# will-rowe/groot

Hardware: AMD Instinct MI355X
Metric: Mreads/s aligned (higher is better)
Workload: dtype u64

## Files before the change

### groot_amd/csrc/hip/ctx.hpp

```cpp
#pragma once

#include <hip/hip_runtime.h>

#include <algorithm>
#include <array>
#include <atomic>
#include <cstdlib>
#include <deque>
#include <map>
#include <memory>
#include <string>
#include <thread>
#include <vector>

#include "device_types.hpp"

using namespace groot;


template <class T> struct DevBuf {
    T *p = nullptr;
    size_t n = 0;
    hipError_t alloc(size_t count)
    {
// ... 245 lines not shown
    DevBuf<uint64_t> d_mask;
    DevBuf<DeviceCounters> d_ctr;
    PinBuf<DeviceCounters> h_ctr;
    PinBuf<groot_trav> h_trav;
    DevBuf<groot_ctrav> d_ctrav;
    PinBuf<groot_ctrav> h_ctrav;
    PinBuf<uint8_t> h_mask;
    PinBuf<uint32_t> h_ckpt;
    DevBuf<uint8_t> d_cmask;
    DevBuf<uint32_t> d_mwords, d_moff, d_ckpt;
    uint32_t n_trav = 0, copied = 0;
    uint64_t n_mask_bytes = 0, copied_bytes = 0;
    bool host_results = false;
    hipEvent_t ev_seed = nullptr;
    hipEvent_t ev_walk = nullptr;
    hipEvent_t ev_h2d0 = nullptr, ev_h2d = nullptr, ev_compute = nullptr, ev_ctr = nullptr, ev_d2h0 = nullptr, ev_d2h = nullptr;
    hipEvent_t ev[14]{};
    groot_counts counts{};
    int status = GROOT_OK;
    std::string status_msg;
    groot_stage_ms ms{};
    SlotCounters ct;
    const uint8_t *seq() const { return input == IN_DEVICE ? ext_seq : d_seq.p; }
    const uint64_t *off() const { return input == IN_DEVICE ? ext_off : d_off.p; }
};

struct WorkSet {
    DevBuf<uint32_t> seed_count, seed_win, perm, perm_count, trav_cnt, tab_idx;
    DevBuf<uint32_t> perm2;
    DevBuf<uint4> packed;
    DevBuf<ReadRec> read_rec;
    DevBuf<uint4> vitem, split_list;
    DevBuf<uint32_t> vcount;
    DevBuf<groot_trav> trav_first;
    DevBuf<uint64_t> mask_first, sketches;
    DevBuf<groot_trav> ovf_trav;
    DevBuf<uint64_t> ovf_mask;
    DevBuf<uint32_t> ovf_cnt;
    hipEvent_t ev_free = nullptr;
    bool used = false;
    Slot *owner = nullptr;
    uint64_t ticket = 0;
};

struct groot_ctx {
    int device = 0;
    std::string err;
    groot_params prm{};
    Knobs kn;
    uint32_t s = 0, k = 0, max_k = 0, l_max = 0, pw_view = 0, pw = 0, n_windows = 0, max_q = 0, band_hash_bits = 0;
    hipEvent_t h2d_last = nullptr;
    Slot *newest = nullptr;
    hipEvent_t last_compute = nullptr;
    hipStream_t own_stream = nullptr, stream = nullptr, astream = nullptr, tstream = nullptr, own_tstream = nullptr, h2d_stream = nullptr, d2h_stream = nullptr;
    bool profiling = false;

    DevBuf<uint32_t> graph_win_end;
    DevBuf<uint4> cn_pre;
    DevBuf<uint64_t> node_l2b;
    DevBuf<uint32_t> win_prefix, edges, win_graph, cn_node,
        band_keys, band_ids;
    DevBuf<ExactEntry> band_hash;
    DevBuf<uint8_t> band_sig;
    DevBuf<uint32_t> band_run;
    DevBuf<uint8_t> bases, q_k, q_l;
    DevBuf<uint16_t> q_min_eq;
    DevBuf<uint64_t> win_sketch;
    DevBuf<unsigned char> node_rec;
// ... 111 lines not shown
```

### groot_amd/csrc/hip/device_types.hpp

```cpp
#pragma once

#include <cstdint>

#include <hip/hip_runtime.h>

#include "groot_hip.h"

namespace groot {

constexpr int kBlock = 256;
constexpr uint32_t kEmpty = 0xFFFFFFFFu;

enum : uint32_t {
    kFlagShortRead = 1u,
    kFlagLongRead = 2u,
    kFlagSeedOverflow = 4u,
    kFlagTravOverflow = 8u,
    kFlagOrdOverflow = 16u,
    kFlagOvfOverflow = 32u,
    kFlagQOverflow = 64u,
};

constexpr uint32_t kIncrCap = 8;
constexpr uint32_t kIncrCapBig = 2048;
// ... 137 lines not shown

struct SeedArgs {
    DeviceIndex ix;
    const uint8_t *seq;
    const uint64_t *seq_off;
    uint32_t n_reads, max_read_len;
    uint32_t lds_read_bytes;
    uint32_t seed_slots;
    uint32_t *seed_count;
    uint32_t *seed_win;
    uint64_t *sketch_out;
    uint32_t *sort_key;
    uint32_t sort_span_bits;
    uint32_t sort_span_shift;
    ReadRec *read_rec;
    uint32_t *q_seen;
    uint32_t *trav_cnt;
    unsigned long long *shards;
    uint32_t *tab_idx;
    uint32_t *tab_hist;
    uint32_t *lsh_list, *lsh_count;
    uint64_t *lsh_sketch;
    uint32_t *dfs_list, *dfs_count;
    uint32_t *long_list, *long_count;
    uint4 *packed;
    uint32_t packed_q;
    uint32_t *todo_list;
    uint32_t *todo_count;
    uint32_t lsh_defer_rows, lsh_cap;
    uint32_t list_stride_dw;
    DeviceCounters *ctr;
};

struct AlignArgs {
    DeviceIndex ix;
    const uint8_t *seq;
    const uint64_t *seq_off;
    uint32_t n_reads, first_read_id;
    uint32_t seed_slots;
    const uint32_t *seed_count;
    const uint32_t *seed_win;
    const uint32_t *perm;
    const ReadRec *read_rec;
    uint32_t no_align, update_weights;
    const void *node_rec;
    uint32_t *attempts;
    groot_trav *trav_first;
    uint64_t *mask_first;
    uint32_t *trav_cnt;
    groot_trav *ovf_trav;
    uint64_t *ovf_mask;
    uint32_t *ovf_cnt;
    uint32_t ovf_cap;
    uint64_t *stk_hdr;
    uint64_t *stk_mask;
    uint32_t n_threads, stk_depth;
    uint32_t lds_stride_dw;
    uint32_t *incr_cnt, *incr_win;
    uint32_t incr_cap;
    uint32_t head_lanes;
    uint32_t round_lanes;
    const uint4 *vitem;
    const uint32_t *vcount;
    uint32_t vcap;
    const uint32_t *n_perm;
    const uint32_t *rest;
    uint32_t rest_lo;
    uint32_t refill;
    DeviceCounters *ctr;
};

struct alignas(16) LeanNode {
    uint32_t seq_off;
    uint32_t seq_len;
    uint32_t deg_kids;
    uint32_t pad;
    uint32_t edges[4];
    uint64_t first32;
    uint64_t mask[3];
};
static_assert(sizeof(LeanNode) == 64, "lean node record is one 64-byte line");
constexpr uint32_t kLeanNo = 0x80000000u;
struct alignas(16) LeanExt {
    uint64_t b[7];
    uint64_t pad;
};
static_assert(sizeof(LeanExt) == 64, "lean node extension is one 64-byte line");
constexpr uint32_t kLeanMaxLen = 256;

struct LeanArgs {
    const LeanNode *nodes;
    const LeanExt *ext;
    const uint32_t *bases2;
    const uint4 *cn_pre2;
    const uint64_t *node_l2b;
    const uint8_t *win_ok;
    const WinRec *win_rec;
    const uint32_t *q_row;
    const uint8_t *seq;
    const uint4 *packed;
    uint32_t packed_q;
    const uint32_t *perm;
    const ReadRec *read_rec;
    uint32_t n_reads, first_read_id, n_windows, k;
    uint32_t update_weights;
    uint32_t lds_stride_dw;
    uint32_t max_len;
    uint32_t *attempts;
    groot_trav *trav_first;
    uint64_t *mask_first;
    uint32_t *trav_cnt;
    uint32_t *left;
    uint32_t *left_cnt;
    uint4 *stk;
    groot_trav *ovf_trav;
    uint64_t *ovf_mask;
    uint32_t *ovf_cnt;
    uint32_t ovf_cap;
    DeviceCounters *ctr;
    const uint4 *path_node;
    const uint32_t *path_text;
    const uint32_t *path_tag;
    const uint32_t *path_nodes;
    const uint64_t *path_tab;
    uint4 *hold;
};

__host__ __device__ inline uint32_t lean_stride_dw(uint32_t max_len) { return (((max_len + 15u) >> 4) + 15u) | 1u; }

#define GROOT_MULTI_SEED 0x90b45d39fb6da1faULL
__host__ __device__ __forceinline__ uint64_t sketch_hash_step(uint64_t h, uint64_t v)
{
    h = (h ^ v) * 0xff51afd7ed558ccdULL;
    return h ^ (h >> 29);
}
#define GROOT_SKETCH_HASH_INIT 0x9E3779B97F4A7C15ULL
__host__ __device__ __forceinline__ uint32_t sig5(uint64_t v) { return (uint32_t)((v * 0xD6E8FEB86659FD93ULL) >> 59); }
constexpr uint32_t kRowSlots = 24, kRowBytes = 16;
__host__ __device__ __forceinline__ uint64_t l2_bloom_bits(uint32_t code16)
{
    const uint32_t x = code16 * 0x9E3779B1u;
    return (1ull << (x >> 26)) | (1ull << ((x >> 20) & 63u));
}
// ... 43 lines not shown
```

### groot_amd/csrc/hip/groot_hip.hip

```cpp
#include <cstring>

#include <hip/hip_runtime.h>
#include <rocprim/rocprim.hpp>

#include <dlfcn.h>

#include <algorithm>
#include <cmath>
#include <cstdarg>
#include <cstdio>
#include <atomic>
#include <chrono>
#include <deque>
#include <iterator>
#include <array>
#include <map>
#include <tuple>
#include <memory>
#include <numeric>
#include <string>
#include <thread>
#include <vector>

#include "../common/cpus.hpp"
// ... 274 lines not shown
    auto sort = [&](void *tmp) {
        return small_blocks ? rocprim::radix_sort_pairs<OrderSortConfig>(tmp, tmp_bytes, c->sort_key.p, c->sort_key_out.p, c->perm_in.p, w->perm.p, s->n_reads,
                                                                         begin_bit, end_bit, c->stream)
                            : rocprim::radix_sort_pairs(tmp, tmp_bytes, c->sort_key.p, c->sort_key_out.p, c->perm_in.p, w->perm.p, s->n_reads, begin_bit, end_bit,
                                                        c->stream);
    };
    HIP_TRY(c, sort(nullptr));
    if (tmp_bytes > c->sort_tmp.n) {
        HIP_TRY(c, hipStreamSynchronize(c->stream));
        HIP_TRY(c, c->sort_tmp.alloc(tmp_bytes + tmp_bytes / 4));
    }
    HIP_TRY(c, sort(c->sort_tmp.p));
    return GROOT_OK;
}

static int launch_align_stage(groot_ctx *c, Slot *s, bool update_weights)
{
    WorkSet *w = &c->ws[s->set];
    AlignArgs a{};
    a.ix = c->dix;
    a.seq = s->seq();
    a.seq_off = s->off();
    a.n_reads = s->n_reads;
    a.first_read_id = s->first_read_id;
    a.seed_slots = c->seed_slots;
    a.seed_count = w->seed_count.p;
    a.seed_win = w->seed_win.p;
    a.perm = w->perm.p;
    a.read_rec = w->read_rec.p;
    a.no_align = c->prm.no_exact_align;
    a.update_weights = update_weights ? 1 : 0;
    a.attempts = c->attempts_ptr;
    a.node_rec = c->node_rec.p;
    a.trav_first = w->trav_first.p;
    a.mask_first = w->mask_first.p;
    a.trav_cnt = w->trav_cnt.p;
    a.ovf_trav = w->ovf_trav.p;
    a.ovf_mask = w->ovf_mask.p;
    a.ovf_cnt = w->ovf_cnt.p;
    a.ovf_cap = c->ovf_cap;
    if (c->vcap) { a.vitem = w->vitem.p; a.vcount = w->vcount.p; a.vcap = c->vcap; }
    a.stk_hdr = c->stk_hdr.p;
    a.stk_mask = c->stk_mask.p;
    uint32_t blocks = std::min<uint32_t>((s->n_reads + kBlock - 1) / kBlock, c->align_threads / kBlock);
    if (c->dfs_frac < kSparseBelow && c->dfs_frac * (double)s->n_reads < 16.0 * (double)(blocks * (kBlock / 64))) blocks = std::max(1u, blocks / 2);
    else if (error_batch(c, s) && blocks >= 4) blocks /= 2;
    if ((s->lean_used || s->path_used) && c->lean_left_frac < 0.25) {
        uint32_t want = (uint32_t)(c->lean_left_frac * 1.25 * (double)s->n_reads / 64.0 / (kBlock / 64)) + 1u;
        blocks = std::max(1u, std::min(blocks, std::max(want, c->n_cu)));
    }
    a.n_threads = blocks * kBlock;
    a.stk_depth = c->stk_depth;
    {
        const uint32_t stride = (2 + 4 * ((s->max_len + 27) / 16)) | 1u;
        a.lds_stride_dw = (size_t)kBlock * stride * 4 <= 64 * 1024 ? stride : 0;
    }
    if (c->tab_capture) {
        a.incr_cnt = c->incr_cnt.p; a.incr_win = c->incr_win.p; a.incr_cap = c->incr_cap;
        HIP_TRY(c, hipMemsetAsync(c->incr_cnt.p, 0, (size_t)s->n_reads * sizeof(uint32_t), c->tstream));
    }
    a.head_lanes = s->mixed_len ? 16u : 0u;
#ifndef GROOT_REFILL_ERR
#define GROOT_REFILL_ERR 48
#endif
#ifndef GROOT_REFILL_MIXED
#define GROOT_REFILL_MIXED 2
#endif
    a.refill = s->mixed_len ? (uint32_t)GROOT_REFILL_MIXED : (error_batch(c, s) ? (uint32_t)GROOT_REFILL_ERR : 64u);
#ifdef GROOT_WORK_COUNTERS
    if (const char *e = getenv("GROOT_DEV_ROUND")) a.round_lanes = (uint32_t)atoi(e);
#endif
    a.ctr = s->d_ctr.p;
    const bool first_pass = s->lean_used || s->path_used;
    const uint32_t lean_stride = lean_stride_dw(s->max_len);
    if (first_pass) {
        LeanArgs l{};
        l.nodes = c->lean_nodes.p; l.ext = c->lean_ext.p; l.bases2 = c->bases2.p; l.cn_pre2 = c->cn_pre2.p; l.win_ok = c->win_ok.p;
        l.win_rec = c->dix.win_rec; l.node_l2b = c->dix.node_l2b; l.q_row = c->q_row.p;
        l.seq = s->seq(); l.packed = s->packed_q ? w->packed.p : nullptr; l.packed_q = s->packed_q; l.perm = w->perm.p; l.read_rec = w->read_rec.p;
        l.n_reads = s->n_reads; l.first_read_id = s->first_read_id; l.n_windows = c->n_windows; l.k = c->k;
        l.update_weights = update_weights ? 1 : 0;
        l.lds_stride_dw = lean_stride; l.max_len = s->max_len;
        l.attempts = c->attempts_ptr;
        l.trav_first = w->trav_first.p; l.mask_first = w->mask_first.p; l.trav_cnt = w->trav_cnt.p;
        l.left = w->perm2.p; l.left_cnt = w->ovf_cnt.p + kOvfShards + 2; l.ctr = s->d_ctr.p;
        l.stk = c->lean_stk.p; l.ovf_trav = w->ovf_trav.p; l.ovf_mask = w->ovf_mask.p; l.ovf_cnt = w->ovf_cnt.p; l.ovf_cap = c->ovf_cap;
        const uint32_t lean_blocks = std::min<uint32_t>((s->n_reads + kBlock - 1) / kBlock, (uint32_t)(c->dfs_frac * 1.05 * (double)s->n_reads / kBlock) + 64u);
        if (s->path_used) {
            l.path_node = c->path_node.p; l.path_text = c->path_text.p; l.path_tag = c->path_tag.p; l.path_nodes = c->path_nodes.p; l.path_tab = c->path_tab.p;
            l.hold = c->path_hold.p;
            launch_align_path(c->pw, l, dim3(lean_blocks), c->astream);
        } else launch_align_lean(c->pw, l, dim3(lean_blocks), c->astream);
        HIP_TRY(c, hipGetLastError());
        a.perm = w->perm2.p;
        a.n_perm = l.left_cnt;
        a.rest = w->perm.p;
        a.rest_lo = lean_blocks * (uint32_t)kBlock;
        if (c->profiling) HIP_TRY(c, hipEventRecord(s->ev[13], c->astream));
        if (c->tstream != c->astream) {
            HIP_TRY(c, hipEventRecord(s->ev_walk, c->astream));
            HIP_TRY(c, hipStreamWaitEvent(c->tstream, s->ev_walk, 0));
        }
    }
    launch_align(c->pw, a, dim3(blocks), c->tstream);
    HIP_TRY(c, hipGetLastError());
    return GROOT_OK;
}

static int launch_order_stage(groot_ctx *c, Slot *s, bool update_weights)
{
    WorkSet *w = &c->ws[s->set];
    const uint32_t n = s->n_reads;
    size_t tmp_bytes = 0;
    if (c->vcap) hipLaunchKernelGGL(split_fix_kernel, dim3(256), dim3(kBlock), 0, c->tstream, w->split_list.p, w->vcount.p, w->vitem.p, w->trav_cnt.p, n, s->d_ctr.p,
                                    w->trav_first.p, w->mask_first.p, c->pw, s->first_read_id);
    HIP_TRY(c, rocprim::exclusive_scan(nullptr, tmp_bytes, w->trav_cnt.p, c->trav_off.p, 0u, n, rocprim::plus<uint32_t>(), c->tstream));
    if (tmp_bytes > c->scan_tmp.n) {
        HIP_TRY(c, hipStreamSynchronize(c->tstream));
        HIP_TRY(c, c->scan_tmp.alloc(tmp_bytes + tmp_bytes / 4));
    }
    HIP_TRY(c, rocprim::exclusive_scan(c->scan_tmp.p, tmp_bytes, w->trav_cnt.p, c->trav_off.p, 0u, n, rocprim::plus<uint32_t>(), c->tstream));
    OrderTabArgs ot{};
    if (c->dix.out_tab) {
        ot.tab_idx = w->tab_idx.p; ot.out_tab = c->dix.out_tab; ot.stride_q = c->dix.out_stride_q; ot.first_read_id = s->first_read_id;
        ot.update_weights = update_weights ? 1 : 0;
        ot.attempts = c->attempts_ptr; ot.q_row = c->q_row.p;
        ot.q_tab = c->dix.w - c->k + 1; ot.n_windows = c->n_windows;
    }
    if (c->profiling) HIP_TRY(c, hipEventRecord(s->ev[9], c->tstream));
    hipLaunchKernelGGL(order_first_kernel, dim3(std::min<uint32_t>((n + kBlock - 1) / kBlock, 2048u)), dim3(kBlock), 0, c->tstream, w->trav_first.p,
                       w->mask_first.p, c->trav_off.p, w->trav_cnt.p, n, s->d_trav.p, s->d_mask.p, s->trav_cap, c->pw,
                       c->pw_view, s->d_ctr.p, ot);
    if (c->profiling) HIP_TRY(c, hipEventRecord(s->ev[10], c->tstream));
    if (c->vcap) hipLaunchKernelGGL(order_split_kernel, dim3(std::min<uint32_t>((c->vcap + kBlock - 1) / kBlock, 256u)), dim3(kBlock), 0, c->tstream, w->vitem.p, w->vcount.p, c->vcap, w->trav_cnt.p,
                                    c->trav_off.p, w->trav_first.p, w->mask_first.p, n, s->first_read_id, s->d_trav.p, s->d_mask.p, s->trav_cap, c->pw, c->pw_view, s->d_ctr.p);
    hipLaunchKernelGGL(order_ovf_kernel, dim3((c->ovf_cap + kBlock - 1) / kBlock, kOvfShards), dim3(kBlock), 0, c->tstream,
                       w->ovf_trav.p, w->ovf_mask.p, w->ovf_cnt.p, c->ovf_cap, c->trav_off.p, s->first_read_id, s->d_trav.p,
                       s->d_mask.p, s->trav_cap, c->pw, c->pw_view, s->d_ctr.p, w->vitem.p, n, w->vcount.p);
    HIP_TRY(c, hipGetLastError());
    if (int rc = counters_assign(c, s)) return rc;
    if (!c->prm.results_on_device) {
        const dim3 g((s->trav_cap + kBlock - 1) / kBlock);
        hipLaunchKernelGGL(mask_words_kernel, g, dim3(kBlock), 0, c->tstream, s->d_trav.p, s->d_ctr.p, s->trav_cap, c->graph_words.p, (uint32_t)c->h_graph_words.size(),
                           s->d_mwords.p);
        size_t tb = 0;
        HIP_TRY(c, rocprim::exclusive_scan(nullptr, tb, s->d_mwords.p, s->d_moff.p, 0u, s->trav_cap, rocprim::plus<uint32_t>(), c->tstream));
        if (tb > c->scan_tmp.n) {
            HIP_TRY(c, hipStreamSynchronize(c->tstream));
            HIP_TRY(c, c->scan_tmp.alloc(tb + tb / 4));
        }
        HIP_TRY(c, rocprim::exclusive_scan(c->scan_tmp.p, tb, s->d_mwords.p, s->d_moff.p, 0u, s->trav_cap, rocprim::plus<uint32_t>(), c->tstream));
        hipLaunchKernelGGL(mask_compact_kernel, g, dim3(kBlock), 0, c->tstream, s->d_trav.p, s->d_mask.p, c->pw_view, s->d_ctr.p, s->trav_cap,
                           c->graph_words.p, (uint32_t)c->h_graph_words.size(), s->d_moff.p, s->d_cmask.p, s->d_ckpt.p);
        if (c->packed_travs) hipLaunchKernelGGL(trav_pack_kernel, g, dim3(kBlock), 0, c->tstream, s->d_trav.p, s->d_ctr.p, s->trav_cap, s->first_read_id, s->d_ctrav.p);
        HIP_TRY(c, hipGetLastError());
    }
    return GROOT_OK;
}


static int run_batch_async(groot_ctx *c, Slot *s, bool update_weights)
{
    WorkSet *w = &c->ws[s->set];
    if (w->used) HIP_TRY(c, hipStreamWaitEvent(c->stream, w->ev_free, 0));
    HIP_TRY(c, hipMemsetAsync(s->d_ctr.p, 0, sizeof(DeviceCounters), c->stream));
    if (c->kn.poison) {
        const size_t n = s->n_reads;
        HIP_TRY(c, hipMemsetAsync(w->seed_count.p, 0, n * sizeof(uint32_t), c->stream));
// ... 1255 lines not shown
```

### groot_amd/csrc/hip/kernels_align.hpp

```cpp
#pragma once

#include "kernels_common.hpp"

namespace groot {


enum : uint32_t { PH_FETCH, PH_SCAN, PH_DFS, PH_WAIT, PH_DONE, PH_FORK, PH_FORKWAIT, PH_JOIN };
#ifndef GROOT_FORK_MIN
#define GROOT_FORK_MIN 3
#endif
constexpr uint32_t kForkMin = GROOT_FORK_MIN;
constexpr uint32_t kClsHelper = 0x1000u;
constexpr uint32_t kCoopMin = 6;
constexpr uint32_t kCoopWant = 0xFFFFFFFEu;
#ifndef GROOT_COOP_MAX_ASK
#define GROOT_COOP_MAX_ASK 8
#endif
constexpr uint32_t kCoopMaxAsk = GROOT_COOP_MAX_ASK;
#ifndef GROOT_TL_LATE_US
#define GROOT_TL_LATE_US 3000
#endif
#ifndef GROOT_WAVE_CHUNK
#define GROOT_WAVE_CHUNK 128
#endif
// ... 670 lines not shown
            if (nb) {
                const uint8_t *gb = ix.bases + rec.seq_off() + coff;
                const uint64_t ga = coff == 0 ? rec.first8() : ld8(gb);
                ok = prefix_ok(ga, cur8, min(nb, 8u));
                for (uint32_t i = 8; ok && i < nb; i += 8)
                    ok = prefix_ok(ld8(gb + i), dfs_chunk(dist + i), nb - i);
            }
            bool backtrack = !ok;
            if (!ok) GROOT_EV(12);
            if (take > 8) GROOT_EV(11);
            if (take > 32) GROOT_EV(21);
            if (ok) {
                dist += nb; coff += nb;
                cur8 = dfs_chunk(dist);
                if (nb == take) {
                    GROOT_EV(13);
                    bool any = false;
#pragma unroll
                    for (int i = 0; i < PW; i++) { mask[i] &= rec.mask(i); any |= mask[i] != 0; }
                    const uint32_t rdeg = rec.deg();
                    if (dist == eff() || rdeg == 0) {
                        if (any && (cls & kClsHelper)) {
                            fk |= 1u << 12; sp = 0; emitted = 1;
                        } else if (any) {
                            GROOT_EV(14);
                            if (ord) GROOT_EV(19);
                            groot_trav t;
                            t.read_id = read_id; t.graph_id = g; t.node = node0; t.offset = noff0;
                            t.ord = (uint16_t)ord;
                            t.flags = (uint8_t)((rc ? GROOT_TRAV_RC : 0u) | (level == 3u ? GROOT_TRAV_START_CLIP : level == 4u ? GROOT_TRAV_END_CLIP : 0u) | (emitted == 0 ? GROOT_TRAV_FIRST : 0));
                            t.reserved = 0;
                            if (ord == 0) {
                                const uint32_t os = (cls & 0x400u) ? a.n_reads + slot : r;
                                a.trav_first[os] = t;
#pragma unroll
                                for (int i = 0; i < PW; i++) a.mask_first[(size_t)os * PW + i] = mask[i];
                            } else {
                                const uint32_t shard = blockIdx.x & (kOvfShards - 1);
                                const uint32_t slot = atomicAdd(&a.ovf_cnt[shard], 1u);
                                if (slot < a.ovf_cap) {
                                    const size_t o = (size_t)shard * a.ovf_cap + slot;
                                    a.ovf_trav[o] = t;
#pragma unroll
                                    for (int i = 0; i < PW; i++) a.ovf_mask[o * PW + i] = mask[i];
                                } else atomicOr(&a.ctr->flags, kFlagOvfOverflow);
                            }
                            if (ord >= 0xFFFFu) atomicOr(&a.ctr->flags, kFlagOrdOverflow);
                            ord++;
#pragma unroll
                            for (int i = 0; i < PW; i++) alns += __popcll(mask[i]);
                            emitted++;
                        }
                        backtrack = true;
                    } else if (!any) backtrack = true;
                    else {
                        const unsigned nextb = (unsigned)cur8 & 0xFF;
                        uint32_t first = kEmpty, more = kEmpty;
                        if (rdeg <= 4) {
#pragma unroll
                            for (int e = 3; e >= 0; e--) {
                                const unsigned cf1 = rec.child_first(e);
                                if ((uint32_t)e < rdeg && (cf1 == 'N' || cf1 == nextb)) { more = first; first = e; }
                            }
                        } else { first = 0; more = 1; }
                        if (first == kEmpty) backtrack = true;
                        else {
                            if (more != kEmpty) {
                                GROOT_EV(15);
                                const size_t si = (size_t)sp * a.n_threads + gtid;
// ... 120 lines not shown
```

### groot_amd/csrc/hip/kernels_lean.hpp

```cpp
#pragma once

#include "kernels_common.hpp"
#include "kernels_path.hpp"

namespace groot {


#ifndef GROOT_LEAN_WAVES
#define GROOT_LEAN_WAVES 5
#endif
constexpr int kLeanWaves = GROOT_LEAN_WAVES;
#ifndef GROOT_LEAN_MAX_ITER
#define GROOT_LEAN_MAX_ITER 96
#endif
constexpr uint32_t kLeanMaxIter = GROOT_LEAN_MAX_ITER;

__device__ __forceinline__ uint64_t lean_lowmask(int n) { return n <= 0 ? 0ull : (n >= 32 ? ~0ull : ((1ull << (2 * n)) - 1ull)); }
__device__ __forceinline__ uint32_t lean_revcomp16(uint32_t v)
{
    uint32_t r = __brev(v);
    r = ((r & 0xAAAAAAAAu) >> 1) | ((r & 0x55555555u) << 1);
    return r ^ 0xAAAAAAAAu;
}
__device__ __forceinline__ uint64_t lean_funnel(uint32_t x0, uint32_t x1, uint32_t x2, uint32_t sh)
// ... 101 lines not shown
    uint32_t si = 1;
    uint32_t done_graph = kEmpty, n_graphs = 1, ord = 0, calls = 1;
    uint32_t alns = 0;
    uint32_t rc = 0, level = 0, eff = len;
    uint32_t sbit = 64;
    auto chunk = [&](uint32_t d) -> uint64_t { return lean_bits64(my, sbit + 2u * d); };
    auto flip = [&]() {
        const uint32_t nd = (len + 15u) >> 4;
        for (uint32_t k2 = 0; 2u * k2 < nd; k2++) {
            const uint32_t x = my[2 + k2], y = my[1 + nd - k2];
            my[2 + k2] = lean_revcomp16(y);
            my[1 + nd - k2] = lean_revcomp16(x);
        }
        rc ^= 1u;
    };
    uint32_t p16 = 0;
    uint64_t need = 0;
    uint32_t pos = 0, sub = 0, lim = 0;
    uint32_t node0 = 0, noff0 = 0, cur = 0, cur_s0 = 0, coff = 0, dist = 0;
    bool cur_long = false;
    uint64_t cur64 = 0, m0 = 0, m1 = 0, m2 = 0;
    uint32_t emitted = 0, sp = 0;
    uint4 *stk = a.stk + (size_t)slot * 4;
    uint32_t t = 0, tend = 0, idx = 0, nbase = 0, tbase = 0, pnn = 0;
    bool pn_need = false;
    uint4 *hold = PATH ? a.hold + (size_t)slot * (3 * kPathHold) : nullptr;
    auto emit = [&]() {
        groot_trav t_;
        t_.read_id = a.first_read_id + r; t_.graph_id = g; t_.node = node0; t_.offset = noff0;
        t_.ord = (uint16_t)ord;
        t_.flags = (uint8_t)((rc ? GROOT_TRAV_RC : 0u) | (level == 3u ? GROOT_TRAV_START_CLIP : level == 4u ? GROOT_TRAV_END_CLIP : 0u) | (emitted == 0u ? GROOT_TRAV_FIRST : 0u));
        t_.reserved = 0;
        if (ord == 0u) {
            a.trav_first[r] = t_;
            a.mask_first[(size_t)r * PW] = m0; a.mask_first[(size_t)r * PW + 1] = m1; a.mask_first[(size_t)r * PW + 2] = m2;
        } else if (PATH) {
            if (ord > kPathHold) { st = ST_DEFER; LEAN_WHY(13); return; }
            uint4 *h = hold + 3u * (ord - 1u);
            h[0] = make_uint4(g, node0, noff0, (uint32_t)t_.ord | ((uint32_t)t_.flags << 16));
            h[1] = make_uint4((uint32_t)m0, (uint32_t)(m0 >> 32), (uint32_t)m1, (uint32_t)(m1 >> 32));
            h[2] = make_uint4((uint32_t)m2, (uint32_t)(m2 >> 32), 0u, 0u);
        } else {
            const uint32_t shard = blockIdx.x & (kOvfShards - 1);
            const uint32_t at = atomicAdd(&a.ovf_cnt[shard], 1u);
            if (at < a.ovf_cap) {
                const size_t o = (size_t)shard * a.ovf_cap + at;
                a.ovf_trav[o] = t_;
                a.ovf_mask[o * PW] = m0; a.ovf_mask[o * PW + 1] = m1; a.ovf_mask[o * PW + 2] = m2;
            } else atomicOr(&a.ctr->flags, kFlagOvfOverflow);
        }
        ord++; emitted++;
        alns += (uint32_t)(__popcll(m0) + __popcll(m1) + __popcll(m2));
    };

    auto verdict = [&](uint32_t bit) -> bool { return si == 1u && (((vbits >> (rc ? 3 : 0)) >> bit) & 1u); };
    auto enter = [&](uint32_t lv) {
        const uint32_t off0 = W[W_OFF0], seed_len = W[W_SLEN];
        bool view = false;
        for (;;) {
            if (lv == 1u) {
                level = 1; view = true;
                if (!verdict(0)) {
                    pos = off0; lim = W[W_L1HI];
                    if (pos < lim) break;
                    lv = 2; continue;
                }
                lv = 3; continue;
            }
// ... 373 lines not shown
```

### groot_amd/csrc/hip/kernels_misc.hpp

```cpp
#pragma once

#include "kernels_common.hpp"

namespace groot {

__global__ __launch_bounds__(kBlock) void lsh_heavy_kernel(SeedArgs a)
{
    __shared__ uint64_t sk_lds[(kBlock / 64) * kLshHeavyMaxS];
    __shared__ uint32_t aux_lds[(kBlock / 64) * (2 * kLshMaxBands + 16)];
    const DeviceIndex &ix = a.ix;
    const uint32_t S = ix.s, maxk = ix.max_k, LB = ix.l_max, n = ix.n_windows;
    const uint32_t sl = S < kRowSlots ? S : kRowSlots, nd = (sl + 5) / 6;
    const uint32_t lane = threadIdx.x & 63, wave = threadIdx.x >> 6;
    uint64_t *m = sk_lds + wave * kLshHeavyMaxS;
    uint32_t *blo = aux_lds + wave * (2 * kLshMaxBands + 16);
    uint32_t *bcum = blo + kLshMaxBands;
    uint32_t *sc = bcum + kLshMaxBands + 1;
    auto wave_sync = []() { __builtin_amdgcn_fence(__ATOMIC_SEQ_CST, "wavefront"); __builtin_amdgcn_wave_barrier(); };
    const uint32_t n_list = min(*a.lsh_count, a.lsh_cap);
    for (uint32_t hi = blockIdx.x * (kBlock / 64) + wave; hi < n_list; hi += gridDim.x * (kBlock / 64)) {
        const uint32_t li = hi;
        const uint32_t e0 = a.lsh_list[li];
        const uint32_t r = e0 & 0x7FFFFFFFu, high = e0 >> 31;
        const uint64_t o0 = a.seq_off[r];
// ... 158 lines not shown
                    graphs++;
                    if (x - lo >= target || x == cnt) { seg[ns++] = x; lo = x; }
                }
                if (ns > 1 && seg[ns - 1] - seg[ns - 2] < kSplitMin / 2) { seg[ns - 2] = seg[ns - 1]; ns--; }
                uint32_t j0 = kEmpty;
                if (ns > 1) {
                    j0 = atomicAdd(&a.vcount[0], ns - 1);
                    if (j0 > a.vcap || ns - 1 > a.vcap - j0) {
                        for (uint32_t j = j0; j < min(j0 + ns - 1, a.vcap); j++) a.vitem[j] = make_uint4(kEmpty, 0, 0, 0);
                        j0 = kEmpty;
                    }
                }
                seg[kSplitMaxItems] = ns; seg[kSplitMaxItems + 1] = j0; seg[kSplitMaxItems + 2] = graphs;
            }
            wave_sync();
            const uint32_t ns = seg[kSplitMaxItems], j0 = seg[kSplitMaxItems + 1];
            if (ns > 1 && j0 != kEmpty) {
                for (uint32_t k = 1 + lane; k < ns; k += 64) a.vitem[j0 + k - 1] = make_uint4(r, seg[k - 1], seg[k], 0);
                if (lane == 0) {
                    const uint32_t si = atomicAdd(&a.vcount[1], 1u);
                    a.split_list[si] = make_uint4(r, j0, ns - 1, 0);
                    if (a.update_weights && seg[kSplitMaxItems + 2] > 1) atomicAdd(&a.ctr->multimapped, 1ull);
                    uint32_t &cf = a.read_rec[r].cnt_flags;
                    cf = (cf & ~kRecCountMask) | seg[0] | kRecSplit;
                }
            }
            wave_sync();
        }
        if (lane == 0) a.read_rec[r].cnt_flags |= flags;
    }
}

__global__ __launch_bounds__(kBlock) void split_fix_kernel(const uint4 *__restrict__ split_list, const uint32_t *__restrict__ vcount, uint4 *__restrict__ vitem,
                                                           uint32_t *__restrict__ trav_cnt, uint32_t n_reads, DeviceCounters *ctr, groot_trav *__restrict__ first,
                                                           uint64_t *__restrict__ mask_first, uint32_t pw, uint32_t first_read_id)
{
    const uint32_t ns = min(vcount[1], kLongListCap);
    for (uint32_t i = blockIdx.x * kBlock + threadIdx.x; i < ns; i += gridDim.x * kBlock) {
        const uint4 sl = split_list[i];
        const uint32_t own = trav_cnt[sl.x];
        uint32_t base = own, first_with = kEmpty;
        for (uint32_t j = sl.y; j < sl.y + sl.z; j++) {
            const uint32_t n = trav_cnt[n_reads + j];
            vitem[j].w = base;
            if (n && first_with == kEmpty) first_with = j;
            base += n;
        }
        if (base > 0xFFFFu) atomicOr(&ctr->flags, kFlagOrdOverflow);
        trav_cnt[sl.x] = base;
        if (!own && first_with != kEmpty) {
            groot_trav t = first[n_reads + first_with];
            t.read_id = first_read_id + sl.x;
            t.ord = 0;
            first[sl.x] = t;
            for (uint32_t w = 0; w < pw; w++) mask_first[(size_t)sl.x * pw + w] = mask_first[(size_t)(n_reads + first_with) * pw + w];
        }
    }
}

__global__ __launch_bounds__(kBlock) void order_split_kernel(const uint4 *__restrict__ vitem, const uint32_t *__restrict__ vcount, uint32_t vcap,
                                                             const uint32_t *__restrict__ trav_cnt, const uint32_t *__restrict__ off, const groot_trav *__restrict__ first,
                                                             const uint64_t *__restrict__ mask_first, uint32_t n_reads, uint32_t first_read_id, groot_trav *__restrict__ out,
                                                             uint64_t *__restrict__ mask_out, uint32_t cap, uint32_t pw_in, uint32_t pw_out, DeviceCounters *ctr)
{
    const uint32_t nv = min(vcount[0], vcap);
    for (uint32_t j = blockIdx.x * kBlock + threadIdx.x; j < nv; j += gridDim.x * kBlock) {
        const uint4 vi = vitem[j];
        if (vi.x == kEmpty || trav_cnt[n_reads + j] == 0) continue;
        const uint32_t i = off[vi.x] + vi.w;
        if (i >= cap) { atomicOr(&ctr->flags, kFlagTravOverflow); continue; }
        groot_trav t = first[n_reads + j];
        t.read_id = first_read_id + vi.x;
        t.ord = (uint16_t)vi.w;
        out[i] = t;
        for (uint32_t w = 0; w < pw_out; w++) mask_out[(size_t)i * pw_out + w] = mask_first[(size_t)(n_reads + j) * pw_in + w];
    }
}

__global__ __launch_bounds__(64) void assign_q_rows_kernel(uint32_t *q_seen, uint32_t *q_row, uint32_t *q_of_row, uint32_t *n_rows, uint32_t cap,
                                                            uint32_t max_q, DeviceCounters *ctr, unsigned long long *shards, uint32_t *long_count,
                                                            uint32_t *todo_count, uint32_t *lsh_count, uint32_t *ovf_cnt)
{
    if (blockIdx.x) return;
    const uint32_t lane = threadIdx.x;
    if (!lane) {
        ctr->long_reads = *long_count;
        *long_count = 0;
        *todo_count = 0;
        if (lsh_count) { ctr->lsh_reads = lsh_count[0]; lsh_count[0] = 0; lsh_count[1] = 0; }
    }
    for (uint32_t i = lane; i < kOvfShards + 3; i += 64) ovf_cnt[i] = 0;
    {
        unsigned long long seeds = 0, most = 0, seeded = 0, tabbed = 0;
        for (uint32_t i = lane; i < kSeedShards; i += 64) {
            unsigned long long *sh = shards + (size_t)i * kSeedShardStride;
            seeds += sh[0];
            most = sh[1] > most ? sh[1] : most;
            seeded += sh[2];
            tabbed += sh[3];
            sh[0] = 0; sh[1] = 0; sh[2] = 0; sh[3] = 0;
        }
        for (int o = 32; o; o >>= 1) {
            seeds += __shfl_xor(seeds, o);
            seeded += __shfl_xor(seeded, o);
            tabbed += __shfl_xor(tabbed, o);
            const unsigned long long other = __shfl_xor(most, o);
            most = other > most ? other : most;
        }
// ... 39 lines not shown
    if (i >= cap || i >= ctr->n_trav) return;
    const groot_trav t = in[i];
    out[i] = groot_ctrav{t.node, t.offset, ((t.read_id - first_read_id) & 0x00FFFFFFu) | ((uint32_t)t.flags << 24)};
}

__global__ __launch_bounds__(kBlock) void add_u32_kernel(uint32_t *__restrict__ dst, const uint32_t *__restrict__ src, size_t n)
{
    for (size_t i = (size_t)blockIdx.x * kBlock + threadIdx.x; i < n; i += (size_t)gridDim.x * kBlock) dst[i] += src[i];
}

__global__ __launch_bounds__(kBlock) void fold_tab_hist_kernel(uint32_t *__restrict__ hist, uint32_t *__restrict__ attempts, const uint32_t *__restrict__ q_row,
                                                               uint32_t q_tab, uint32_t n_windows, const DeviceCounters *ctr, uint32_t update_weights)
{
    const bool live = update_weights && !(ctr->flags & (kFlagSeedOverflow | kFlagQOverflow));
    const uint32_t row = live ? q_row[q_tab] : kEmpty;
    for (uint32_t w = blockIdx.x * kBlock + threadIdx.x; w < n_windows; w += gridDim.x * kBlock) {
        const uint32_t v = hist[w];
        if (!v) continue;
        hist[w] = 0;
        if (row != kEmpty) atomicAdd(&attempts[(size_t)row * n_windows + w], v);
    }
}


struct OrderTabArgs {
    const uint32_t *tab_idx;
    const uint4 *out_tab;
    uint32_t stride_q, first_read_id;
    uint32_t update_weights;
    uint32_t *attempts;
    const uint32_t *q_row;
    uint32_t q_tab, n_windows;
};
__global__ __launch_bounds__(kBlock) void order_first_kernel(const groot_trav *first, const uint64_t *mask_first, const uint32_t *off,
                                                           const uint32_t *cnt, uint32_t n, groot_trav *out, uint64_t *mask_out,
                                                           uint32_t cap, uint32_t pw_in, uint32_t pw_out, DeviceCounters *ctr, OrderTabArgs t)
{
    __shared__ unsigned long long red[4];
    unsigned long long alns = 0, mapped = 0, multimapped = 0, seeds = 0;
    const bool live = !(ctr->flags & (kFlagSeedOverflow | kFlagQOverflow));
    if (blockIdx.x == 0 && threadIdx.x == 0 && n) ctr->n_trav = off[n - 1] + cnt[n - 1];
    for (uint32_t r = blockIdx.x * kBlock + threadIdx.x; r < n; r += gridDim.x * kBlock) {
    const uint32_t tw = t.tab_idx ? t.tab_idx[r] : kEmpty;
    const uint32_t ti = tw == kEmpty ? kEmpty : tw & ((1u << kOutIdxBits) - 1u);
    const bool count_here = (t.update_weights & 1u) && !(tw & kTabCounted);
    const bool seeds_here = tw != kEmpty && (tw & kTabSeedsHere);
    uint32_t ns = 0;
    if (ti != kEmpty && live) {
        const uint32_t nt = cnt[r], i = off[r];
        const bool fits = i < cap && nt <= cap - i;
        if (!fits) atomicOr(&ctr->flags, kFlagTravOverflow);
        const uint32_t row = t.update_weights ? t.q_row[t.q_tab] : 0u;
        uint32_t n_ent = nt ? nt : 1u;
        for (uint32_t j = 0; j < n_ent; j++) {
            const uint4 *e = t.out_tab + (size_t)(ti + j) * t.stride_q;
            uint4 h = e[0];
            if (j == 0) { n_ent += h.z >> 20; h.z &= 0xFFFFFu; }
            const uint4 x = e[1];
            const uint4 y = pw_out > 1 ? e[2] : make_uint4(0, 0, 0, 0);
            if (count_here) {
                if (x.x != kEmpty) atomicAdd(&t.attempts[(size_t)row * t.n_windows + x.x], 1u);
                if (x.y != kEmpty) atomicAdd(&t.attempts[(size_t)row * t.n_windows + x.y], 1u);
            }
            if (seeds_here) ns += (h.w >> 10) & 7u;
            if (j == 0) { mapped += (h.w >> 9) & 1u; multimapped += (h.w >> 8) & 1u; }
            if (j < nt) {
                alns += __popc(x.z) + __popc(x.w) + __popc(y.x) + __popc(y.y) + __popc(y.z) + __popc(y.w);
                if (pw_out > 3) {
                    const uint32_t *ew = reinterpret_cast<const uint32_t *>(e) + kOutHdrDw;
                    for (uint32_t w = 6; w < 2 * pw_out; w++) alns += __popc(ew[w]);
                }
            }
            if (!fits || j >= nt) continue;
            groot_trav tr;
            tr.read_id = t.first_read_id + r; tr.graph_id = h.z; tr.node = h.x; tr.offset = h.y;
            tr.ord = (uint16_t)j; tr.flags = (uint8_t)h.w; tr.reserved = 0;
            uint64_t *mo = mask_out + (size_t)(i + j) * pw_out;
            static_assert(sizeof(groot_trav) == 20, "record is five dwords");
            uint32_t tw5[5];
            __builtin_memcpy(tw5, &tr, 20);
            uint32_t *po = reinterpret_cast<uint32_t *>(out + i + j);
#pragma unroll
            for (int d = 0; d < 5; d++) __builtin_nontemporal_store(tw5[d], po + d);
            __builtin_nontemporal_store((uint64_t)x.z | ((uint64_t)x.w << 32), mo);
            if (pw_out > 1) __builtin_nontemporal_store((uint64_t)y.x | ((uint64_t)y.y << 32), mo + 1);
            if (pw_out > 2) __builtin_nontemporal_store((uint64_t)y.z | ((uint64_t)y.w << 32), mo + 2);
            const uint32_t *ew = reinterpret_cast<const uint32_t *>(e) + kOutHdrDw;
            for (uint32_t w = 3; w < pw_out; w++) mo[w] = (uint64_t)ew[2 * w] | ((uint64_t)ew[2 * w + 1] << 32);
        }
        if (seeds_here) seeds += ns;
    } else if (ti == kEmpty && cnt[r] != 0) {
        const uint32_t i = off[r];
        if (i >= cap) atomicOr(&ctr->flags, kFlagTravOverflow);
        else {
            out[i] = first[r];
            for (uint32_t w = 0; w < pw_out; w++) mask_out[(size_t)i * pw_out + w] = mask_first[(size_t)r * pw_in + w];
        }
    }
    }
    if (!t.tab_idx) return;
    alns = block_sum(alns, red);
    mapped = block_sum(mapped, red);
    multimapped = block_sum(multimapped, red);
    seeds = block_sum(seeds, red);
    if (threadIdx.x == 0) {
        if (alns) atomicAdd(&ctr->alignments, alns);
        if (seeds) atomicAdd(&ctr->seeds, seeds);
        if (t.update_weights) {
            if (mapped) atomicAdd(&ctr->mapped, mapped);
            if (multimapped) atomicAdd(&ctr->multimapped, multimapped);
        }
    }
}

__global__ __launch_bounds__(kBlock) void order_ovf_kernel(const groot_trav *ovf, const uint64_t *ovf_mask, const uint32_t *ovf_cnt,
                                                         uint32_t ovf_cap, const uint32_t *off, uint32_t first_read_id, groot_trav *out,
                                                         uint64_t *mask_out, uint32_t cap, uint32_t pw_in, uint32_t pw_out,
                                                         DeviceCounters *ctr, const uint4 *vitem, uint32_t n_reads, uint32_t *vcount)
{
    const uint32_t shard = blockIdx.y;
    const uint32_t slot = blockIdx.x * kBlock + threadIdx.x;
    if (!slot && !shard) { vcount[0] = 0; vcount[1] = 0; }
    if (slot >= min(ovf_cnt[shard], ovf_cap)) return;
    const size_t o = (size_t)shard * ovf_cap + slot;
    groot_trav t = ovf[o];
    uint32_t rid = t.read_id - first_read_id, ord = t.ord;
    if (rid >= n_reads) {
        const uint4 vi = vitem[rid - n_reads];
        rid = vi.x; ord += vi.w;
// ... 37 lines not shown
```

### groot_amd/csrc/hip/open.hip

```cpp
#include <hip/hip_runtime.h>

#include <algorithm>
#include <chrono>
#include <cstdio>
#include <cstring>
#include <memory>
#include <numeric>
#include <string>
#include <thread>
#include <vector>

#include "../common/cpus.hpp"
#include "../common/view_check.hpp"
#include "counters.hpp"
#include "ctx.hpp"
#include "index_tables.hpp"
#include "kernels_open.hpp"
#include "kernels_path.hpp"
#include "launch.hpp"
#include "open.hpp"

using namespace groot;

static int text_pass(groot_ctx *c, const uint8_t *seqs, const uint32_t *owner, uint32_t n, uint32_t len, uint8_t *differs, uint32_t *cnt_flags,
// ... 519 lines not shown
        std::unique_ptr<Slot> s(new Slot());
        for (hipEvent_t *e : {&s->ev_seed, &s->ev_walk, &s->ev_h2d0, &s->ev_h2d, &s->ev_compute, &s->ev_ctr, &s->ev_d2h0, &s->ev_d2h}) HIP_TRY(c, hipEventCreate(e));
        for (auto &e : s->ev) HIP_TRY(c, hipEventCreate(&e));
        c->slots.push_back(std::move(s));
    }
    return GROOT_OK;
}

static int alloc_work_buffers(groot_ctx *c)
{
    const uint32_t R = c->prm.max_batch_reads, s = c->s;
    HIP_TRY(c, c->sort_key.alloc(R));
    HIP_TRY(c, c->sort_key_out.alloc(R));
    HIP_TRY(c, c->long_list.alloc(kLongListCap));
    HIP_TRY(c, c->long_count.alloc(4));
    HIP_TRY(c, hipMemset(c->long_count.p, 0, 4 * sizeof(uint32_t)));
    {
        std::vector<uint32_t> iota(R);
        std::iota(iota.begin(), iota.end(), 0u);
        HIP_TRY(c, upload(c->perm_in, iota.data(), iota.size()));
    }
    if (int rc = alloc_seed_slots(c, c->prm.max_seeds_per_read)) return rc;
    c->vcap = c->kn.small_buffers ? 8u : std::max<uint32_t>(4096, R / 4);
    for (WorkSet &w : c->ws) {
        HIP_TRY(c, w.seed_count.alloc(R));
        HIP_TRY(c, w.read_rec.alloc(R));
        HIP_TRY(c, w.perm.alloc(R));
        HIP_TRY(c, w.perm_count.alloc(4));
        if (c->lean || c->path) {
            HIP_TRY(c, w.perm2.alloc(R));
            HIP_TRY(c, w.packed.alloc((size_t)R * (c->prm.max_read_len <= 128 ? 2 : 4)));
        }
        if (c->prm.keep_sketches) HIP_TRY(c, w.sketches.alloc((size_t)R * s));
        HIP_TRY(c, w.trav_first.alloc((size_t)R + c->vcap));
        HIP_TRY(c, w.mask_first.alloc(((size_t)R + c->vcap) * c->pw));
        HIP_TRY(c, w.trav_cnt.alloc((size_t)R + c->vcap));
        HIP_TRY(c, w.vitem.alloc(std::max<uint32_t>(c->vcap, 1)));
        HIP_TRY(c, w.split_list.alloc(kLongListCap));
        HIP_TRY(c, w.vcount.alloc(4));
        HIP_TRY(c, hipMemset(w.vcount.p, 0, 4 * sizeof(uint32_t)));
    }
    HIP_TRY(c, c->trav_off.alloc(R));
    if (c->lean || c->path) HIP_TRY(c, c->lean_stk.alloc((size_t)R * 4));
    if (c->path) HIP_TRY(c, c->path_hold.alloc((size_t)R * 3 * kPathHold));
    for (WorkSet &w : c->ws) {
        HIP_TRY(c, w.ovf_cnt.alloc(kOvfShards + 3));
        HIP_TRY(c, hipMemset(w.ovf_cnt.p, 0, (kOvfShards + 3) * sizeof(uint32_t)));
    }
    if (int rc = alloc_ovf(c, c->kn.small_buffers ? 2u : std::max<uint32_t>(256, R / kOvfShards / 4))) return rc;
    int n_cu = 256;
    (void)hipDeviceGetAttribute(&n_cu, hipDeviceAttributeMultiprocessorCount, c->device);
    c->n_cu = (uint32_t)std::max(n_cu, 1);
    uint32_t per_cu = c->pw > 3 ? kAlignWavesWide : kAlignWaves;
    c->align_threads = std::min<uint32_t>(((R + kBlock - 1) / kBlock) * kBlock, (uint32_t)std::max(n_cu, 1) * per_cu * kBlock);
    c->stk_depth = c->prm.max_read_len;
    HIP_TRY(c, c->stk_hdr.alloc((size_t)c->stk_depth * c->align_threads));
    HIP_TRY(c, c->stk_mask.alloc((size_t)c->stk_depth * c->align_threads * c->pw));
    if (c->l_max <= kLshMaxBands) {
#ifndef GROOT_LSH_DEFER_ROWS
#define GROOT_LSH_DEFER_ROWS 64
#endif
        c->lsh_defer_rows = GROOT_LSH_DEFER_ROWS;
        c->lsh_cap = c->kn.small_buffers ? 4u : std::max<uint32_t>(4096, R / 4);
        HIP_TRY(c, c->lsh_list.alloc(c->lsh_cap));
        HIP_TRY(c, c->lsh_count.alloc(4));
        HIP_TRY(c, hipMemset(c->lsh_count.p, 0, 4 * sizeof(uint32_t)));
        HIP_TRY(c, c->lsh_sketch.alloc((size_t)c->lsh_cap * s));
    }
// ... 288 lines not shown
```

Before: 2481.

## Interleave first traversal record and mask into one padded uint4 record

Result: faster. 2545 (median of 6 runs) (+2.6%).

```diff
diff --git a/groot_amd/csrc/hip/ctx.hpp b/groot_amd/csrc/hip/ctx.hpp
--- a/groot_amd/csrc/hip/ctx.hpp
+++ b/groot_amd/csrc/hip/ctx.hpp
@@ -301,8 +301,8 @@
     DevBuf<ReadRec> read_rec;
     DevBuf<uint4> vitem, split_list;
     DevBuf<uint32_t> vcount;
-    DevBuf<groot_trav> trav_first;
-    DevBuf<uint64_t> mask_first, sketches;
+    DevBuf<uint4> first_rec;
+    DevBuf<uint64_t> sketches;
     DevBuf<groot_trav> ovf_trav;
     DevBuf<uint64_t> ovf_mask;
     DevBuf<uint32_t> ovf_cnt;
diff --git a/groot_amd/csrc/hip/device_types.hpp b/groot_amd/csrc/hip/device_types.hpp
--- a/groot_amd/csrc/hip/device_types.hpp
+++ b/groot_amd/csrc/hip/device_types.hpp
@@ -193,6 +193,31 @@
     DeviceCounters *ctr;
 };
 
+__host__ __device__ constexpr uint32_t first_rec_q(uint32_t pw) { return pw <= 5u ? 4u : 8u; }
+__device__ __forceinline__ const uint64_t *first_rec_mask(const uint4 *rec, uint32_t q, size_t slot) { return reinterpret_cast<const uint64_t *>(rec + slot * q) + 3; }
+__device__ __forceinline__ groot_trav first_rec_trav(const uint4 *rec, uint32_t q, size_t slot)
+{
+    static_assert(sizeof(groot_trav) == 20, "record is five dwords");
+    const uint4 a = rec[slot * q];
+    const uint32_t d[5] = {a.x, a.y, a.z, a.w, reinterpret_cast<const uint32_t *>(rec + slot * q)[4]};
+    groot_trav t;
+    __builtin_memcpy(&t, d, 20);
+    return t;
+}
+template <int PW>
+__device__ __forceinline__ void first_rec_store(uint4 *rec, size_t slot, const groot_trav &t, const uint64_t *mask)
+{
+    uint32_t d[5];
+    __builtin_memcpy(d, &t, 20);
+    uint4 *o = rec + slot * first_rec_q(PW);
+    o[0] = make_uint4(d[0], d[1], d[2], d[3]);
+    o[1] = make_uint4(d[4], 0u, (uint32_t)mask[0], (uint32_t)(mask[0] >> 32));
+    uint64_t *m = reinterpret_cast<uint64_t *>(o) + 3;
+#pragma unroll
+    for (int i = 1; i + 1 < PW; i += 2) o[(i + 3) / 2] = make_uint4((uint32_t)mask[i], (uint32_t)(mask[i] >> 32), (uint32_t)mask[i + 1], (uint32_t)(mask[i + 1] >> 32));
+    if ((PW & 1) == 0) m[PW - 1] = mask[PW - 1];
+}
+
 struct AlignArgs {
     DeviceIndex ix;
     const uint8_t *seq;
@@ -206,8 +231,7 @@
     uint32_t no_align, update_weights;
     const void *node_rec;
     uint32_t *attempts;
-    groot_trav *trav_first;
-    uint64_t *mask_first;
+    uint4 *first_rec;
     uint32_t *trav_cnt;
     groot_trav *ovf_trav;
     uint64_t *ovf_mask;
@@ -268,8 +292,7 @@
     uint32_t lds_stride_dw;
     uint32_t max_len;
     uint32_t *attempts;
-    groot_trav *trav_first;
-    uint64_t *mask_first;
+    uint4 *first_rec;
     uint32_t *trav_cnt;
     uint32_t *left;
     uint32_t *left_cnt;
diff --git a/groot_amd/csrc/hip/groot_hip.hip b/groot_amd/csrc/hip/groot_hip.hip
--- a/groot_amd/csrc/hip/groot_hip.hip
+++ b/groot_amd/csrc/hip/groot_hip.hip
@@ -330,8 +330,7 @@
     a.update_weights = update_weights ? 1 : 0;
     a.attempts = c->attempts_ptr;
     a.node_rec = c->node_rec.p;
-    a.trav_first = w->trav_first.p;
-    a.mask_first = w->mask_first.p;
+    a.first_rec = w->first_rec.p;
     a.trav_cnt = w->trav_cnt.p;
     a.ovf_trav = w->ovf_trav.p;
     a.ovf_mask = w->ovf_mask.p;
@@ -380,7 +379,7 @@
         l.update_weights = update_weights ? 1 : 0;
         l.lds_stride_dw = lean_stride; l.max_len = s->max_len;
         l.attempts = c->attempts_ptr;
-        l.trav_first = w->trav_first.p; l.mask_first = w->mask_first.p; l.trav_cnt = w->trav_cnt.p;
+        l.first_rec = w->first_rec.p; l.trav_cnt = w->trav_cnt.p;
         l.left = w->perm2.p; l.left_cnt = w->ovf_cnt.p + kOvfShards + 2; l.ctr = s->d_ctr.p;
         l.stk = c->lean_stk.p; l.ovf_trav = w->ovf_trav.p; l.ovf_mask = w->ovf_mask.p; l.ovf_cnt = w->ovf_cnt.p; l.ovf_cap = c->ovf_cap;
         const uint32_t lean_blocks = std::min<uint32_t>((s->n_reads + kBlock - 1) / kBlock, (uint32_t)(c->dfs_frac * 1.05 * (double)s->n_reads / kBlock) + 64u);
@@ -411,7 +410,7 @@
     const uint32_t n = s->n_reads;
     size_t tmp_bytes = 0;
     if (c->vcap) hipLaunchKernelGGL(split_fix_kernel, dim3(256), dim3(kBlock), 0, c->tstream, w->split_list.p, w->vcount.p, w->vitem.p, w->trav_cnt.p, n, s->d_ctr.p,
-                                    w->trav_first.p, w->mask_first.p, c->pw, s->first_read_id);
+                                    w->first_rec.p, c->pw, s->first_read_id);
     HIP_TRY(c, rocprim::exclusive_scan(nullptr, tmp_bytes, w->trav_cnt.p, c->trav_off.p, 0u, n, rocprim::plus<uint32_t>(), c->tstream));
     if (tmp_bytes > c->scan_tmp.n) {
         HIP_TRY(c, hipStreamSynchronize(c->tstream));
@@ -426,12 +425,12 @@
         ot.q_tab = c->dix.w - c->k + 1; ot.n_windows = c->n_windows;
     }
     if (c->profiling) HIP_TRY(c, hipEventRecord(s->ev[9], c->tstream));
-    hipLaunchKernelGGL(order_first_kernel, dim3(std::min<uint32_t>((n + kBlock - 1) / kBlock, 2048u)), dim3(kBlock), 0, c->tstream, w->trav_first.p,
-                       w->mask_first.p, c->trav_off.p, w->trav_cnt.p, n, s->d_trav.p, s->d_mask.p, s->trav_cap, c->pw,
+    hipLaunchKernelGGL(order_first_kernel, dim3(std::min<uint32_t>((n + kBlock - 1) / kBlock, 2048u)), dim3(kBlock), 0, c->tstream, w->first_rec.p,
+                       c->trav_off.p, w->trav_cnt.p, n, s->d_trav.p, s->d_mask.p, s->trav_cap, c->pw,
                        c->pw_view, s->d_ctr.p, ot);
     if (c->profiling) HIP_TRY(c, hipEventRecord(s->ev[10], c->tstream));
     if (c->vcap) hipLaunchKernelGGL(order_split_kernel, dim3(std::min<uint32_t>((c->vcap + kBlock - 1) / kBlock, 256u)), dim3(kBlock), 0, c->tstream, w->vitem.p, w->vcount.p, c->vcap, w->trav_cnt.p,
-                                    c->trav_off.p, w->trav_first.p, w->mask_first.p, n, s->first_read_id, s->d_trav.p, s->d_mask.p, s->trav_cap, c->pw, c->pw_view, s->d_ctr.p);
+                                    c->trav_off.p, w->first_rec.p, n, s->first_read_id, s->d_trav.p, s->d_mask.p, s->trav_cap, c->pw, c->pw_view, s->d_ctr.p);
     hipLaunchKernelGGL(order_ovf_kernel, dim3((c->ovf_cap + kBlock - 1) / kBlock, kOvfShards), dim3(kBlock), 0, c->tstream,
                        w->ovf_trav.p, w->ovf_mask.p, w->ovf_cnt.p, c->ovf_cap, c->trav_off.p, s->first_read_id, s->d_trav.p,
                        s->d_mask.p, s->trav_cap, c->pw, c->pw_view, s->d_ctr.p, w->vitem.p, n, w->vcount.p);
diff --git a/groot_amd/csrc/hip/kernels_align.hpp b/groot_amd/csrc/hip/kernels_align.hpp
--- a/groot_amd/csrc/hip/kernels_align.hpp
+++ b/groot_amd/csrc/hip/kernels_align.hpp
@@ -726,9 +726,7 @@
                             t.reserved = 0;
                             if (ord == 0) {
                                 const uint32_t os = (cls & 0x400u) ? a.n_reads + slot : r;
-                                a.trav_first[os] = t;
-#pragma unroll
-                                for (int i = 0; i < PW; i++) a.mask_first[(size_t)os * PW + i] = mask[i];
+                                first_rec_store<PW>(a.first_rec, os, t, mask);
                             } else {
                                 const uint32_t shard = blockIdx.x & (kOvfShards - 1);
                                 const uint32_t slot = atomicAdd(&a.ovf_cnt[shard], 1u);
diff --git a/groot_amd/csrc/hip/kernels_lean.hpp b/groot_amd/csrc/hip/kernels_lean.hpp
--- a/groot_amd/csrc/hip/kernels_lean.hpp
+++ b/groot_amd/csrc/hip/kernels_lean.hpp
@@ -157,8 +157,8 @@
         t_.flags = (uint8_t)((rc ? GROOT_TRAV_RC : 0u) | (level == 3u ? GROOT_TRAV_START_CLIP : level == 4u ? GROOT_TRAV_END_CLIP : 0u) | (emitted == 0u ? GROOT_TRAV_FIRST : 0u));
         t_.reserved = 0;
         if (ord == 0u) {
-            a.trav_first[r] = t_;
-            a.mask_first[(size_t)r * PW] = m0; a.mask_first[(size_t)r * PW + 1] = m1; a.mask_first[(size_t)r * PW + 2] = m2;
+            const uint64_t mk[3] = {m0, m1, m2};
+            first_rec_store<PW>(a.first_rec, r, t_, mk);
         } else if (PATH) {
             if (ord > kPathHold) { st = ST_DEFER; LEAN_WHY(13); return; }
             uint4 *h = hold + 3u * (ord - 1u);
diff --git a/groot_amd/csrc/hip/kernels_misc.hpp b/groot_amd/csrc/hip/kernels_misc.hpp
--- a/groot_amd/csrc/hip/kernels_misc.hpp
+++ b/groot_amd/csrc/hip/kernels_misc.hpp
@@ -214,8 +214,8 @@
 }
 
 __global__ __launch_bounds__(kBlock) void split_fix_kernel(const uint4 *__restrict__ split_list, const uint32_t *__restrict__ vcount, uint4 *__restrict__ vitem,
-                                                           uint32_t *__restrict__ trav_cnt, uint32_t n_reads, DeviceCounters *ctr, groot_trav *__restrict__ first,
-                                                           uint64_t *__restrict__ mask_first, uint32_t pw, uint32_t first_read_id)
+                                                           uint32_t *__restrict__ trav_cnt, uint32_t n_reads, DeviceCounters *ctr, uint4 *__restrict__ first_rec,
+                                                           uint32_t pw, uint32_t first_read_id)
 {
     const uint32_t ns = min(vcount[1], kLongListCap);
     for (uint32_t i = blockIdx.x * kBlock + threadIdx.x; i < ns; i += gridDim.x * kBlock) {
@@ -231,18 +231,21 @@
         if (base > 0xFFFFu) atomicOr(&ctr->flags, kFlagOrdOverflow);
         trav_cnt[sl.x] = base;
         if (!own && first_with != kEmpty) {
-            groot_trav t = first[n_reads + first_with];
-            t.read_id = first_read_id + sl.x;
-            t.ord = 0;
-            first[sl.x] = t;
-            for (uint32_t w = 0; w < pw; w++) mask_first[(size_t)sl.x * pw + w] = mask_first[(size_t)(n_reads + first_with) * pw + w];
+            const uint32_t q = first_rec_q(pw);
+            uint4 *to = first_rec + (size_t)sl.x * q;
+            const uint4 *from = first_rec + (size_t)(n_reads + first_with) * q;
+            uint4 h0 = from[0], h1 = from[1];
+            h0.x = first_read_id + sl.x;
+            h1.x &= 0xFFFF0000u;
+            to[0] = h0; to[1] = h1;
+            for (uint32_t w = 2; w < q; w++) to[w] = from[w];
         }
     }
 }
 
 __global__ __launch_bounds__(kBlock) void order_split_kernel(const uint4 *__restrict__ vitem, const uint32_t *__restrict__ vcount, uint32_t vcap,
-                                                             const uint32_t *__restrict__ trav_cnt, const uint32_t *__restrict__ off, const groot_trav *__restrict__ first,
-                                                             const uint64_t *__restrict__ mask_first, uint32_t n_reads, uint32_t first_read_id, groot_trav *__restrict__ out,
+                                                             const uint32_t *__restrict__ trav_cnt, const uint32_t *__restrict__ off, const uint4 *__restrict__ first_rec,
+                                                             uint32_t n_reads, uint32_t first_read_id, groot_trav *__restrict__ out,
                                                              uint64_t *__restrict__ mask_out, uint32_t cap, uint32_t pw_in, uint32_t pw_out, DeviceCounters *ctr)
 {
     const uint32_t nv = min(vcount[0], vcap);
@@ -251,11 +254,13 @@
         if (vi.x == kEmpty || trav_cnt[n_reads + j] == 0) continue;
         const uint32_t i = off[vi.x] + vi.w;
         if (i >= cap) { atomicOr(&ctr->flags, kFlagTravOverflow); continue; }
-        groot_trav t = first[n_reads + j];
+        const uint32_t q = first_rec_q(pw_in);
+        groot_trav t = first_rec_trav(first_rec, q, n_reads + j);
+        const uint64_t *mf = first_rec_mask(first_rec, q, n_reads + j);
         t.read_id = first_read_id + vi.x;
         t.ord = (uint16_t)vi.w;
         out[i] = t;
-        for (uint32_t w = 0; w < pw_out; w++) mask_out[(size_t)i * pw_out + w] = mask_first[(size_t)(n_reads + j) * pw_in + w];
+        for (uint32_t w = 0; w < pw_out; w++) mask_out[(size_t)i * pw_out + w] = mf[w];
     }
 }
 
@@ -361,7 +366,7 @@
     const uint32_t *q_row;
     uint32_t q_tab, n_windows;
 };
-__global__ __launch_bounds__(kBlock) void order_first_kernel(const groot_trav *first, const uint64_t *mask_first, const uint32_t *off,
+__global__ __launch_bounds__(kBlock) void order_first_kernel(const uint4 *first_rec, const uint32_t *off,
                                                            const uint32_t *cnt, uint32_t n, groot_trav *out, uint64_t *mask_out,
                                                            uint32_t cap, uint32_t pw_in, uint32_t pw_out, DeviceCounters *ctr, OrderTabArgs t)
 {
@@ -419,11 +424,20 @@
         }
         if (seeds_here) seeds += ns;
     } else if (ti == kEmpty && cnt[r] != 0) {
+        const uint32_t q = first_rec_q(pw_in);
+        const uint4 *rec = first_rec + (size_t)r * q;
+        const uint4 ra = rec[0], rb = rec[1], rc = pw_out > 1 ? rec[2] : make_uint4(0, 0, 0, 0);
         const uint32_t i = off[r];
         if (i >= cap) atomicOr(&ctr->flags, kFlagTravOverflow);
         else {
-            out[i] = first[r];
-            for (uint32_t w = 0; w < pw_out; w++) mask_out[(size_t)i * pw_out + w] = mask_first[(size_t)r * pw_in + w];
+            uint32_t *po = reinterpret_cast<uint32_t *>(out + i);
+            po[0] = ra.x; po[1] = ra.y; po[2] = ra.z; po[3] = ra.w; po[4] = rb.x;
+            uint64_t *mo = mask_out + (size_t)i * pw_out;
+            mo[0] = (uint64_t)rb.z | ((uint64_t)rb.w << 32);
+            if (pw_out > 1) mo[1] = (uint64_t)rc.x | ((uint64_t)rc.y << 32);
+            if (pw_out > 2) mo[2] = (uint64_t)rc.z | ((uint64_t)rc.w << 32);
+            const uint64_t *mf = first_rec_mask(first_rec, q, r);
+            for (uint32_t w = 3; w < pw_out; w++) mo[w] = mf[w];
         }
     }
     }
diff --git a/groot_amd/csrc/hip/open.hip b/groot_amd/csrc/hip/open.hip
--- a/groot_amd/csrc/hip/open.hip
+++ b/groot_amd/csrc/hip/open.hip
@@ -575,8 +575,7 @@
             HIP_TRY(c, w.packed.alloc((size_t)R * (c->prm.max_read_len <= 128 ? 2 : 4)));
         }
         if (c->prm.keep_sketches) HIP_TRY(c, w.sketches.alloc((size_t)R * s));
-        HIP_TRY(c, w.trav_first.alloc((size_t)R + c->vcap));
-        HIP_TRY(c, w.mask_first.alloc(((size_t)R + c->vcap) * c->pw));
+        HIP_TRY(c, w.first_rec.alloc(((size_t)R + c->vcap) * first_rec_q(c->pw)));
         HIP_TRY(c, w.trav_cnt.alloc((size_t)R + c->vcap));
         HIP_TRY(c, w.vitem.alloc(std::max<uint32_t>(c->vcap, 1)));
         HIP_TRY(c, w.split_list.alloc(kLongListCap));
```
